# rcelha/rio-rs

Hardware: NVIDIA H100
Metric: placements/sec (higher is better)
Workload: dtype u32

## Files before the change

rio_rs_b200/csrc/k_trie.cu:

```cuda
#include "kernels.cuh"
#include "spec.cuh"
#include "bounded_tail.cuh"

#include <cstdlib>

namespace rio {

namespace {

#define RIO_COUNT_LAUNCH(L) do { if ((L).launch_counter) ++*(L).launch_counter; } while (0)

constexpr int kTrieThreads = 256;
constexpr uint32_t kMaxLevels = 16;

__constant__ uint32_t c_lvl_s0[kMaxLevels];
__constant__ uint32_t c_lvl_m2[kMaxLevels];
__constant__ uint32_t c_lvl_h2[kMaxLevels];

__device__ __forceinline__ uint32_t smem_u32(const void *p) { return (uint32_t)__cvta_generic_to_shared(p); }

__device__ __forceinline__ void stage_blob_tma(void *smem_dst, const void *gsrc, uint32_t bytes, unsigned long long *bar) {
    if (threadIdx.x == 0) {
        asm volatile("mbarrier.init.shared::cta.b64 [%0], 1;" ::"r"(smem_u32(bar)) : "memory");
        asm volatile("fence.mbarrier_init.release.cluster;" ::: "memory");
    }
    __syncthreads();
    if (threadIdx.x == 0) {
        asm volatile("mbarrier.arrive.expect_tx.shared::cta.b64 _, [%0], %1;" ::"r"(smem_u32(bar)), "r"(bytes) : "memory");
        for (uint32_t off = 0; off < bytes; off += 32768u) {
            const uint32_t len = min(32768u, bytes - off);
            asm volatile("cp.async.bulk.shared::cluster.global.mbarrier::complete_tx::bytes [%0], [%1], %2, [%3];"
                         ::"r"(smem_u32(reinterpret_cast<unsigned char *>(smem_dst) + off)),
                           "l"(reinterpret_cast<const unsigned char *>(gsrc) + off), "r"(len), "r"(smem_u32(bar))
                         : "memory");
        }
    }
    uint32_t done = 0;
    while (!done) {
        asm volatile("{\n\t.reg .pred p;\n\tmbarrier.try_wait.parity.shared::cta.b64 p, [%1], %2;\n\tselp.u32 %0, 1, 0, p;\n\t}"
                     : "=r"(done) : "r"(smem_u32(bar)), "r"(0u) : "memory");
    }
}

__device__ __forceinline__ uint32_t walk_step(uint32_t off, uint32_t sel) {
    uint32_t r;
    asm("mad.lo.u32 %0, %1, 2, %2;" : "=r"(r) : "r"(off), "r"(sel));
    return r;
}

template <int BITS>
__device__ __forceinline__ uint32_t trie_leaf_index(ObjHash o, const uint32_t *__restrict__ tab32, uint32_t bits_rt) {
    uint32_t i = 1;
    if (BITS > 0) {
#pragma unroll
        for (int l = 0; l < BITS; l++) {
            const uint32_t u = contest_u(o, c_lvl_s0[l], c_lvl_m2[l], c_lvl_h2[l]);
            i = 2 * i + (u > tab32[i] ? 1u : 0u);
        }
    } else {
        for (uint32_t l = 0; l < bits_rt; l++) {
            const uint32_t u = contest_u(o, c_lvl_s0[l], c_lvl_m2[l], c_lvl_h2[l]);
            i = 2 * i + (u > tab32[i] ? 1u : 0u);
        }
    }
    return i;
}

__device__ __forceinline__ uint32_t trie_resolve_leaf(ObjHash o, uint32_t leaf, const unsigned char *__restrict__ blob) {
    if ((int32_t)leaf > -2) return leaf;
    uint32_t w = leaf;
    for (;;) {
        const unsigned char *p = blob + (w & 0x7FFFFFFFu);
        const uint4 r = *reinterpret_cast<const uint4 *>(p);
        const uint2 nn = *reinterpret_cast<const uint2 *>(p + 16);
        if (contest_u(o, r.x, r.y, r.z) <= r.w) return nn.x;
        if ((int32_t)nn.y >= 0) return nn.y;
        w = nn.y;
    }
}

struct TrieSmem {
    const uint32_t *tab32;
    const unsigned char *blob;
    uint32_t *hist;
};

template <bool SMEM>
__device__ __forceinline__ TrieSmem trie_stage(const TrieDev &t, uint32_t hist_bins) {
    extern __shared__ __align__(128) unsigned char smem_trie[];
    constexpr bool in_smem = SMEM;
    TrieSmem s;
    uint32_t off = 0;
    if (in_smem) {
        s.tab32 = reinterpret_cast<const uint32_t *>(smem_trie);
        s.blob = smem_trie;
        off = t.blob_bytes;
    } else {
        const unsigned char *g = reinterpret_cast<const unsigned char *>(t.blob);
        s.tab32 = reinterpret_cast<const uint32_t *>(g);
        s.blob = g;
    }
    s.hist = reinterpret_cast<uint32_t *>(smem_trie + off);
    for (uint32_t j = threadIdx.x; j < hist_bins; j += blockDim.x) s.hist[j] = 0;
    unsigned long long *bar = reinterpret_cast<unsigned long long *>(smem_trie + off + ((hist_bins * 4u + 15u) & ~15u));
    if (in_smem) stage_blob_tma(smem_trie, t.blob, t.blob_bytes, bar);
    else __syncthreads();
    return s;
}

template <int BITS, int OPT, int MODE, bool SMEM, int MINB = (SMEM ? 5 : 3)>
__global__ void __launch_bounds__(kTrieThreads, MINB)
k_assign_trie(const uint64_t *__restrict__ keys, uint64_t n, TrieDev t, uint32_t *__restrict__ out_idx, uint32_t *__restrict__ counters,
              uint32_t hist_bins, unsigned long long *__restrict__ moved, const __grid_constant__ BoundedTail tail) {
    static_assert(OPT % 2 == 0, "two objects per 128-bit load");
    constexpr bool in_smem = SMEM;
    constexpr int SEG = OPT / 2;
    const uint64_t tile_objs = (uint64_t)kTrieThreads * OPT;
    const uint64_t n_tiles = (n + tile_objs - 1) / tile_objs;
    unsigned long long n_moved = 0;
    ulonglong2 kk[SEG];
    auto load_tile = [&](uint64_t tile) {
        const uint64_t f0 = tile * tile_objs + 2 * threadIdx.x;
        if ((tile + 1) * tile_objs <= n) {
            const ulonglong2 *src = reinterpret_cast<const ulonglong2 *>(keys + f0);
#pragma unroll
            for (int g = 0; g < SEG; g++) kk[g] = __ldg(src + g * kTrieThreads);
            return;
        }
#pragma unroll
        for (int g = 0; g < SEG; g++) {
            const uint64_t f = f0 + (uint64_t)g * (2 * kTrieThreads);
            kk[g] = make_ulonglong2(0, 0);
            if (f + 1 < n) kk[g] = __ldg(reinterpret_cast<const ulonglong2 *>(keys + f));
            else if (f < n) kk[g].x = __ldg(keys + f);
        }
    };
    const TrieSmem s = trie_stage<SMEM>(t, hist_bins);
    asm volatile("griddepcontrol.launch_dependents;" ::: "memory");
    asm volatile("griddepcontrol.wait;" ::: "memory");
    if (blockIdx.x < n_tiles) load_tile(blockIdx.x);
    for (uint64_t tile = blockIdx.x; tile < n_tiles; tile += gridDim.x) {
        const uint64_t base = tile * tile_objs;
        const bool full_tile = base + tile_objs <= n;
        ObjHash o[OPT];
#pragma unroll
        for (int g = 0; g < SEG; g++) {
            o[2 * g] = obj_hash(kk[g].x);
            o[2 * g + 1] = obj_hash(kk[g].y);
        }
        if (tile + gridDim.x < n_tiles) load_tile(tile + gridDim.x);
        uint32_t leaf[OPT];
        if (in_smem) {
            const unsigned char *tb = reinterpret_cast<const unsigned char *>(s.tab32);
            uint32_t off[OPT];
#pragma unroll
            for (int k = 0; k < OPT; k++) off[k] = 4;
            if (BITS > 0) {
                constexpr int TOP = BITS >= 3 ? 3 : 0;
                if (TOP) {
#pragma unroll
                    for (int k = 0; k < OPT; k++) {
                        const bool c0 = contest_u(o[k], c_lvl_s0[0], c_lvl_m2[0], c_lvl_h2[0]) > t.top[1];
                        const bool c1 = contest_u(o[k], c_lvl_s0[1], c_lvl_m2[1], c_lvl_h2[1]) > (c0 ? t.top[3] : t.top[2]);
                        const uint32_t t2 = c0 ? (c1 ? t.top[7] : t.top[6]) : (c1 ? t.top[5] : t.top[4]);
                        const bool c2 = contest_u(o[k], c_lvl_s0[2], c_lvl_m2[2], c_lvl_h2[2]) > t2;
                        off[k] = 32u + (c0 ? 16u : 0u) + (c1 ? 8u : 0u) + (c2 ? 4u : 0u);
                    }
                }
#pragma unroll
                for (int l = TOP; l < BITS; l++) {
#pragma unroll
                    for (int k = 0; k < OPT; k++) {
                        const uint32_t u = contest_u(o[k], c_lvl_s0[l], c_lvl_m2[l], c_lvl_h2[l]);
                        const uint32_t thr = *reinterpret_cast<const uint32_t *>(tb + off[k]);
                        off[k] = walk_step(off[k], u > thr ? 4u : 0u);
                    }
                }
            } else {
                for (uint32_t l = 0; l < t.bits; l++) {
#pragma unroll
                    for (int k = 0; k < OPT; k++) {
                        const uint32_t u = contest_u(o[k], c_lvl_s0[l], c_lvl_m2[l], c_lvl_h2[l]);
                        const uint32_t thr = *reinterpret_cast<const uint32_t *>(tb + off[k]);
                        off[k] = walk_step(off[k], u > thr ? 4u : 0u);
                    }
                }
            }
#pragma unroll
            for (int k = 0; k < OPT; k++) leaf[k] = *reinterpret_cast<const uint32_t *>(tb + off[k]);
        } else {
#pragma unroll
            for (int k = 0; k < OPT; k++) leaf[k] = __ldg(s.tab32 + trie_leaf_index<0>(o[k], s.tab32, t.bits));
        }
        uint32_t nid[OPT];
#pragma unroll
        for (int k = 0; k < OPT; k++) nid[k] = trie_resolve_leaf(o[k], leaf[k], s.blob);
        if (MODE == 0 && full_tile) {
            uint2 *dst = reinterpret_cast<uint2 *>(out_idx + base + 2 * threadIdx.x);
#pragma unroll
            for (int g = 0; g < SEG; g++) dst[g * kTrieThreads] = make_uint2(nid[2 * g], nid[2 * g + 1]);
            if (counters && nid[0] != kNone) {
                if (hist_bins) {
#pragma unroll
                    for (int k = 0; k < OPT; k++) atomicAdd(&s.hist[nid[k]], 1u);
                } else {
#pragma unroll
                    for (int k = 0; k < OPT; k++) atomicAdd(&counters[nid[k]], 1u);
                }
            }
            continue;
        }
#pragma unroll
        for (int g = 0; g < SEG; g++) {
            const uint64_t first = base + (uint64_t)g * (2 * kTrieThreads) + 2 * threadIdx.x;
            if (first >= n) continue;
            const bool two = first + 1 < n;
            if (MODE == 1) {
                uint2 old = make_uint2(kNone, kNone);
                if (two) old = *reinterpret_cast<const uint2 *>(out_idx + first);
                else old.x = out_idx[first];
                const bool c0 = old.x != nid[2 * g], c1 = two && old.y != nid[2 * g + 1];
                if (c0 | c1) {
                    if (two) *reinterpret_cast<uint2 *>(out_idx + first) = make_uint2(nid[2 * g], nid[2 * g + 1]);
                    else out_idx[first] = nid[2 * g];
                }
                n_moved += (unsigned)c0 + (unsigned)c1;
            } else {
                if (two) *reinterpret_cast<uint2 *>(out_idx + first) = make_uint2(nid[2 * g], nid[2 * g + 1]);
                else out_idx[first] = nid[2 * g];
            }
            if (counters) {
                if (hist_bins) {
                    if (nid[2 * g] != kNone) atomicAdd(&s.hist[nid[2 * g]], 1u);
                    if (two && nid[2 * g + 1] != kNone) atomicAdd(&s.hist[nid[2 * g + 1]], 1u);
                } else {
                    if (nid[2 * g] != kNone) atomicAdd(&counters[nid[2 * g]], 1u);
                    if (two && nid[2 * g + 1] != kNone) atomicAdd(&counters[nid[2 * g + 1]], 1u);
                }
            }
        }
    }
    if (MODE == 1) {
#pragma unroll
        for (int sh = 16; sh > 0; sh >>= 1) n_moved += __shfl_xor_sync(0xFFFFFFFFu, n_moved, sh);
        if ((threadIdx.x & 31) == 0 && n_moved) atomicAdd(moved, n_moved);
    }
    if (hist_bins && counters) {
        __syncthreads();
        for (uint32_t j = threadIdx.x; j < hist_bins; j += blockDim.x) { const uint32_t v = s.hist[j]; if (v) atomicAdd(&counters[j], v); }
    }
    if (MODE == 0 && tail.enabled) {
        __shared__ uint32_t s_last;
        __threadfence();
        __syncthreads();
        if (threadIdx.x == 0) s_last = atomicAdd(tail.ticket, 1u) == gridDim.x - 1;
        __syncthreads();
        if (s_last) {
            if (threadIdx.x == 0) *tail.ticket = 0;
            __threadfence();
            exchange_and_check_block(tail, counters);
        }
    }
}

template <bool SMEM>
__global__ void __launch_bounds__(kTrieThreads, 4)
k_assign_trie_sel(const uint64_t *__restrict__ keys, const uint32_t *__restrict__ sel, uint64_t n_sel, TrieDev t, uint32_t *__restrict__ out_idx,
                  uint32_t *__restrict__ counters, uint32_t hist_bins) {
    const TrieSmem s = trie_stage<SMEM>(t, hist_bins);
    for (uint64_t q = (uint64_t)blockIdx.x * blockDim.x + threadIdx.x; q < n_sel; q += (uint64_t)gridDim.x * blockDim.x) {
        const uint32_t oi = __ldg(sel + q);
        const ObjHash o = obj_hash(__ldg(keys + oi));
        const uint32_t i = trie_leaf_index<0>(o, s.tab32, t.bits);
        const uint32_t nid = trie_resolve_leaf(o, s.tab32[i], s.blob);
        out_idx[oi] = nid;
        if (counters && nid != kNone) { if (hist_bins) atomicAdd(&s.hist[nid], 1u); else atomicAdd(&counters[nid], 1u); }
    }
    if (hist_bins && counters) {
        __syncthreads();
        for (uint32_t j = threadIdx.x; j < hist_bins; j += blockDim.x) { const uint32_t v = s.hist[j]; if (v) atomicAdd(&counters[j], v); }
    }
}

template <bool SMEM>
__global__ void __launch_bounds__(kTrieThreads, 4)
k_dir_reassign_trie(DirDev dir, TrieDev t, unsigned long long *__restrict__ moved) {
    const TrieSmem s = trie_stage<SMEM>(t, 0);
    const uint4 *slots = reinterpret_cast<const uint4 *>(dir.slots);
    const uint64_t cap = dir.mask + 1;
    unsigned long long n_moved = 0;
    for (uint64_t i = (uint64_t)blockIdx.x * blockDim.x + threadIdx.x; i < cap; i += (uint64_t)gridDim.x * blockDim.x) {
        const uint4 v = slots[i];
        const unsigned long long key = ((unsigned long long)v.y << 32) | v.x;
        if (key == kEmptyKey || v.z == kNone) continue;
        const ObjHash o = obj_hash(key);
        const uint32_t li = trie_leaf_index<0>(o, s.tab32, t.bits);
        const uint32_t nid = trie_resolve_leaf(o, s.tab32[li], s.blob);
        if (nid != v.z) { reinterpret_cast<uint32_t *>(&dir.slots[i].val)[0] = nid; n_moved++; }
    }
#pragma unroll
    for (int sh = 16; sh > 0; sh >>= 1) n_moved += __shfl_xor_sync(0xFFFFFFFFu, n_moved, sh);
    if ((threadIdx.x & 31) == 0 && n_moved) atomicAdd(moved, n_moved);
}

constexpr uint32_t kTrieSmemBudget = 200u * 1024u;

struct TrieLaunchShape { uint32_t hist_bins; uint32_t in_smem; size_t smem; int ctas_per_sm; };
TrieLaunchShape trie_shape(const TrieDev &t, bool want_hist, uint32_t n_total, int want_ctas) {
    TrieLaunchShape sh{};
    sh.hist_bins = (want_hist && n_total <= 8192) ? n_total : 0;
    const size_t tail = ((size_t)sh.hist_bins * 4 + 15) / 16 * 16 + 16;
    sh.in_smem = (t.blob_bytes + tail <= kTrieSmemBudget) ? 1u : 0u;
    sh.smem = (sh.in_smem ? t.blob_bytes : 0) + tail;
    int c = want_ctas;
    while (c > 1 && (size_t)c * (sh.smem + 1024) > 227u * 1024u) c--;
    sh.ctas_per_sm = c;
    return sh;
}

bool g_lvl_uploaded[64] = {};

}

void trie_upload_level_constants(int device) {
    if (device >= 0 && device < 64 && g_lvl_uploaded[device]) return;
    uint32_t s0[kMaxLevels], m2[kMaxLevels], h2[kMaxLevels];
    for (uint32_t l = 0; l < kMaxLevels; l++) {
        const ContestRec r = contest_rec(level_seed(l));
        s0[l] = r.s0; m2[l] = r.m2; h2[l] = r.h2;
    }
    cudaMemcpyToSymbol(c_lvl_s0, s0, sizeof s0);
    cudaMemcpyToSymbol(c_lvl_m2, m2, sizeof m2);
    cudaMemcpyToSymbol(c_lvl_h2, h2, sizeof h2);
    if (device >= 0 && device < 64) g_lvl_uploaded[device] = true;
}

uint64_t trie_wave_objects(int sm_count) { return (uint64_t)sm_count * 5 * kTrieThreads * 4; }

#define RIO_TRIE_LAUNCH(KERNEL, GRID, SMEM, ...)                                                                       \
    do {                                                                                                               \
        static bool attr_set[64] = {};    \
        int dev__ = 0;                                                                                                 \
        cudaGetDevice(&dev__);                                                                                         \
        if (dev__ < 0 || dev__ >= 64 || !attr_set[dev__]) {                                                            \
            cudaFuncSetAttribute(KERNEL, cudaFuncAttributeMaxDynamicSharedMemorySize, (int)kTrieSmemBudget + 1024);    \
            if (dev__ >= 0 && dev__ < 64) attr_set[dev__] = true;                                                      \
        }                                                                                                              \
        KERNEL<<<(GRID), kTrieThreads, (SMEM), L.stream>>>(__VA_ARGS__);                                               \
    } while (0)

#define RIO_TRIE_LAUNCH_PDL(KERNEL, GRID, SMEM, ...)                                                                   \
    do {                                                                                                               \
        static bool attr_set[64] = {};                                                                                 \
        static const bool pdl = [] { const char *e = getenv("RIO_TRIE_PDL"); return !(e && e[0] == '0'); }();          \
        int dev__ = 0;                                                                                                 \
        cudaGetDevice(&dev__);                                                                                         \
        if (dev__ < 0 || dev__ >= 64 || !attr_set[dev__]) {                                                            \
            cudaFuncSetAttribute(KERNEL, cudaFuncAttributeMaxDynamicSharedMemorySize, (int)kTrieSmemBudget + 1024);    \
            if (dev__ >= 0 && dev__ < 64) attr_set[dev__] = true;                                                      \
        }                                                                                                              \
        cudaLaunchConfig_t cfg__ = {};                                                                                 \
        cfg__.gridDim = dim3((unsigned)(GRID)); cfg__.blockDim = dim3(kTrieThreads);                                   \
        cfg__.dynamicSmemBytes = (SMEM); cfg__.stream = L.stream;                                                      \
        cudaLaunchAttribute at__[1];                                                                                   \
        at__[0].id = cudaLaunchAttributeProgrammaticStreamSerialization;                                               \
        at__[0].val.programmaticStreamSerializationAllowed = 1;                                                        \
        cfg__.attrs = at__; cfg__.numAttrs = pdl ? 1 : 0;                                                              \
        cudaLaunchKernelEx(&cfg__, KERNEL, __VA_ARGS__);                                                               \
    } while (0)

void launch_assign_trie(const Launch &L, const uint64_t *d_keys, uint64_t n, const TrieDev &t, uint32_t *d_out_idx, uint32_t *d_counters,
                        const uint32_t *d_sel, uint64_t n_sel, uint32_t n_total, const BoundedTail *tail) {
    BoundedTail no_tail{};
    const BoundedTail &tl = tail ? *tail : no_tail;
    const uint64_t n_work = d_sel ? n_sel : n;
    if (!n_work) return;
    if (d_sel) {
        const TrieLaunchShape sh = trie_shape(t, d_counters != nullptr, n_total, 4);
        const uint64_t blocks = (n_work + kTrieThreads - 1) / kTrieThreads, cap = (uint64_t)L.sm_count * sh.ctas_per_sm;
        const int grid = (int)(blocks < cap ? blocks : cap);
        if (sh.in_smem) RIO_TRIE_LAUNCH(k_assign_trie_sel<true>, grid, sh.smem, d_keys, d_sel, n_work, t, d_out_idx, d_counters, sh.hist_bins);
        else RIO_TRIE_LAUNCH(k_assign_trie_sel<false>, grid, sh.smem, d_keys, d_sel, n_work, t, d_out_idx, d_counters, sh.hist_bins);
    } else {
        constexpr int OPT = 4;
#ifdef RIO_ASSIGN_TUNING
        if (const char *tn = getenv("RIO_TRIE_TUNE")) {
            const int code = atoi(tn);
            auto go = [&](auto kern, int opt, int minb) {
                const TrieLaunchShape sh2 = trie_shape(t, d_counters != nullptr, n_total, minb);
                const uint64_t tiles2 = (n_work + (uint64_t)kTrieThreads * opt - 1) / ((uint64_t)kTrieThreads * opt), cap2 = (uint64_t)L.sm_count * sh2.ctas_per_sm;
                cudaFuncSetAttribute(kern, cudaFuncAttributeMaxDynamicSharedMemorySize, (int)kTrieSmemBudget + 1024);
                kern<<<(int)(tiles2 < cap2 ? tiles2 : cap2), kTrieThreads, sh2.smem, L.stream>>>(d_keys, n_work, t, d_out_idx, d_counters, sh2.hist_bins, nullptr, tl);
            };
            bool done = true;
            switch (code) {
                case 25: go(k_assign_trie<12, 2, 0, true, 5>, 2, 5); break;
                case 28: go(k_assign_trie<12, 2, 0, true, 8>, 2, 8); break;
                case 44: go(k_assign_trie<12, 4, 0, true, 4>, 4, 4); break;
                case 45: go(k_assign_trie<12, 4, 0, true, 5>, 4, 5); break;
                case 63: go(k_assign_trie<12, 6, 0, true, 3>, 6, 3); break;
                case 64: go(k_assign_trie<12, 6, 0, true, 4>, 6, 4); break;
                case 83: go(k_assign_trie<12, 8, 0, true, 3>, 8, 3); break;
                default: done = false;
            }
            if (done && t.bits == 12) { RIO_COUNT_LAUNCH(L); return; }
        }
#endif
        const TrieLaunchShape sh = trie_shape(t, d_counters != nullptr, n_total, 5);
        uint64_t cap = (uint64_t)L.sm_count * sh.ctas_per_sm;
        if (L.spare_ctas > 0 && cap > (uint64_t)L.spare_ctas + 1) cap -= (uint64_t)L.spare_ctas;
        const uint64_t tiles = (n_work + (uint64_t)kTrieThreads * OPT - 1) / ((uint64_t)kTrieThreads * OPT);
        const int grid = (int)(tiles < cap ? tiles : cap);
        unsigned long long *no_moved = nullptr;
        if (!sh.in_smem) RIO_TRIE_LAUNCH_PDL((k_assign_trie<0, OPT, 0, false>), grid, sh.smem, d_keys, n_work, t, d_out_idx, d_counters, sh.hist_bins, no_moved, tl);
        else if (t.bits == 12) RIO_TRIE_LAUNCH_PDL((k_assign_trie<12, OPT, 0, true>), grid, sh.smem, d_keys, n_work, t, d_out_idx, d_counters, sh.hist_bins, no_moved, tl);
        else RIO_TRIE_LAUNCH_PDL((k_assign_trie<0, OPT, 0, true>), grid, sh.smem, d_keys, n_work, t, d_out_idx, d_counters, sh.hist_bins, no_moved, tl);
    }
    RIO_COUNT_LAUNCH(L);
}

void launch_reassign_trie(const Launch &L, const uint64_t *d_keys, uint64_t n, const TrieDev &t, uint32_t *d_idx, uint32_t *d_counters,
                          uint32_t n_total, unsigned long long *d_moved) {
    if (!n) return;
    constexpr int OPT = 4;
 const TrieLaunchShape sh = trie_shape(t, d_counters != nullptr, n_total, 5);
    const uint64_t tiles = (n + (uint64_t)kTrieThreads * OPT - 1) / ((uint64_t)kTrieThreads * OPT), cap = (uint64_t)L.sm_count * sh.ctas_per_sm;
    const int grid = (int)(tiles < cap ? tiles : cap);
    if (!sh.in_smem) RIO_TRIE_LAUNCH((k_assign_trie<0, OPT, 1, false>), grid, sh.smem, d_keys, n, t, d_idx, d_counters, sh.hist_bins, d_moved, BoundedTail{});
    else if (t.bits == 12) RIO_TRIE_LAUNCH((k_assign_trie<12, OPT, 1, true>), grid, sh.smem, d_keys, n, t, d_idx, d_counters, sh.hist_bins, d_moved, BoundedTail{});
    else RIO_TRIE_LAUNCH((k_assign_trie<0, OPT, 1, true>), grid, sh.smem, d_keys, n, t, d_idx, d_counters, sh.hist_bins, d_moved, BoundedTail{});
    RIO_COUNT_LAUNCH(L);
}

void launch_dir_reassign_trie(const Launch &L, const DirDev &dir, const TrieDev &t, unsigned long long *d_moved) {
    const TrieLaunchShape sh = trie_shape(t, false, 0, 4);
    const uint64_t blocks = (dir.mask + 1 + kTrieThreads - 1) / kTrieThreads, cap = (uint64_t)L.sm_count * sh.ctas_per_sm;
    const int grid = (int)(blocks < cap ? blocks : cap);
    if (sh.in_smem) RIO_TRIE_LAUNCH(k_dir_reassign_trie<true>, grid, sh.smem, dir, t, d_moved);
    else RIO_TRIE_LAUNCH(k_dir_reassign_trie<false>, grid, sh.smem, dir, t, d_moved);
    RIO_COUNT_LAUNCH(L);
}

}
```

Measured before the change: 148.3 billion.

## Replicate mid trie levels per lane in smem to kill bank conflicts; use 1024-thread CTAs

Trie levels 6-9 are copied into shared memory replicated 32-wide, one copy per lane. Lookups at those levels then hit each lane's own bank instead of colliding on a few hot nodes. The kernel now runs 1024-thread CTAs at one CTA per SM. The compare switches to >= with h2-1 so a carry-based descend instruction can be used, and the chain resolve becomes a batched loop across objects. The costs are extra smem for the replicas, a copy step at kernel start, and lower CTA-level occupancy; the launch API also gains a rep argument.

```diff
diff --git a/rio_rs_b200/csrc/k_trie.cu b/rio_rs_b200/csrc/k_trie.cu
--- a/rio_rs_b200/csrc/k_trie.cu
+++ b/rio_rs_b200/csrc/k_trie.cu
@@ -2,6 +2,7 @@
 #include "spec.cuh"
 #include "bounded_tail.cuh"
 
+#include <algorithm>
 #include <cstdlib>
 
 namespace rio {
@@ -11,7 +12,13 @@
 #define RIO_COUNT_LAUNCH(L) do { if ((L).launch_counter) ++*(L).launch_counter; } while (0)
 
 constexpr int kTrieThreads = 256;
+constexpr int kWalkThreads = 1024;
+constexpr int kWalkCtas = 1;
 constexpr uint32_t kMaxLevels = 16;
+constexpr uint32_t kRepFirst = 6;
+constexpr uint32_t kRepMax = 4;
+__host__ __device__ constexpr uint32_t rep_bytes(uint32_t levels) { return ((1u << (kRepFirst + levels)) - (1u << kRepFirst)) * 128u; }
+constexpr int default_rep(int bits) { return bits <= (int)kRepFirst ? 0 : bits - (int)kRepFirst < (int)kRepMax ? bits - (int)kRepFirst : (int)kRepMax; }
 
 __constant__ uint32_t c_lvl_s0[kMaxLevels];
 __constant__ uint32_t c_lvl_m2[kMaxLevels];
@@ -42,9 +49,9 @@
     }
 }
 
-__device__ __forceinline__ uint32_t walk_step(uint32_t off, uint32_t sel) {
+__device__ __forceinline__ uint32_t descend(uint32_t i, uint32_t u1, uint32_t t3) {
     uint32_t r;
-    asm("mad.lo.u32 %0, %1, 2, %2;" : "=r"(r) : "r"(off), "r"(sel));
+    asm("{\n\t.reg .u32 d;\n\tsub.cc.u32 d, %1, %2;\n\taddc.u32 %0, %3, %3;\n\t}" : "=r"(r) : "r"(u1), "r"(t3), "r"(i));
     return r;
 }
 
@@ -54,13 +61,13 @@
     if (BITS > 0) {
 #pragma unroll
         for (int l = 0; l < BITS; l++) {
-            const uint32_t u = contest_u(o, c_lvl_s0[l], c_lvl_m2[l], c_lvl_h2[l]);
-            i = 2 * i + (u > tab32[i] ? 1u : 0u);
+            const uint32_t u1 = contest_u(o, c_lvl_s0[l], c_lvl_m2[l], c_lvl_h2[l]);
+            i = 2 * i + (u1 >= tab32[i] ? 1u : 0u);
         }
     } else {
         for (uint32_t l = 0; l < bits_rt; l++) {
-            const uint32_t u = contest_u(o, c_lvl_s0[l], c_lvl_m2[l], c_lvl_h2[l]);
-            i = 2 * i + (u > tab32[i] ? 1u : 0u);
+            const uint32_t u1 = contest_u(o, c_lvl_s0[l], c_lvl_m2[l], c_lvl_h2[l]);
+            i = 2 * i + (u1 >= tab32[i] ? 1u : 0u);
         }
     }
     return i;
@@ -79,43 +86,58 @@
     }
 }
 
+extern __shared__ __align__(128) unsigned char smem_trie[];
+
+__device__ __forceinline__ uint32_t lds_u32(uint32_t byte_off) { return *reinterpret_cast<const uint32_t *>(smem_trie + byte_off); }
+
 struct TrieSmem {
     const uint32_t *tab32;
     const unsigned char *blob;
     uint32_t *hist;
+    uint32_t rep_lane;
 };
 
 template <bool SMEM>
-__device__ __forceinline__ TrieSmem trie_stage(const TrieDev &t, uint32_t hist_bins) {
-    extern __shared__ __align__(128) unsigned char smem_trie[];
+__device__ __forceinline__ TrieSmem trie_stage(const TrieDev &t, uint32_t hist_bins, uint32_t rep = 0) {
     constexpr bool in_smem = SMEM;
     TrieSmem s;
     uint32_t off = 0;
     if (in_smem) {
         s.tab32 = reinterpret_cast<const uint32_t *>(smem_trie);
         s.blob = smem_trie;
-        off = t.blob_bytes;
+        off = t.blob_bytes + rep_bytes(rep);
     } else {
         const unsigned char *g = reinterpret_cast<const unsigned char *>(t.blob);
         s.tab32 = reinterpret_cast<const uint32_t *>(g);
         s.blob = g;
     }
+    s.rep_lane = t.blob_bytes + (threadIdx.x & 31u) * 4u - (1u << kRepFirst) * 128u;
     s.hist = reinterpret_cast<uint32_t *>(smem_trie + off);
     for (uint32_t j = threadIdx.x; j < hist_bins; j += blockDim.x) s.hist[j] = 0;
     unsigned long long *bar = reinterpret_cast<unsigned long long *>(smem_trie + off + ((hist_bins * 4u + 15u) & ~15u));
     if (in_smem) stage_blob_tma(smem_trie, t.blob, t.blob_bytes, bar);
     else __syncthreads();
+    if (in_smem && rep) {
+        uint4 *dst = reinterpret_cast<uint4 *>(smem_trie + t.blob_bytes);
+        const uint32_t *src = s.tab32 + (1u << kRepFirst);
+        for (uint32_t q = threadIdx.x; q < rep_bytes(rep) / 16u; q += blockDim.x) {
+            const uint32_t v = src[q >> 3];
+            dst[q] = make_uint4(v, v, v, v);
+        }
+        __syncthreads();
+    }
     return s;
 }
 
-template <int BITS, int OPT, int MODE, bool SMEM, int MINB = (SMEM ? 5 : 3)>
-__global__ void __launch_bounds__(kTrieThreads, MINB)
+template <int BITS, int OPT, int MODE, bool SMEM, int NT = kWalkThreads, int MINB = kWalkCtas, int REP = default_rep(BITS)>
+__global__ void __launch_bounds__(NT, MINB)
 k_assign_trie(const uint64_t *__restrict__ keys, uint64_t n, TrieDev t, uint32_t *__restrict__ out_idx, uint32_t *__restrict__ counters,
-              uint32_t hist_bins, unsigned long long *__restrict__ moved, const __grid_constant__ BoundedTail tail) {
+              uint32_t hist_bins, uint32_t rep, unsigned long long *__restrict__ moved, const __grid_constant__ BoundedTail tail) {
     static_assert(OPT % 2 == 0, "two objects per 128-bit load");
+    static_assert(BITS == 0 || BITS >= 3 + REP, "the unrolled walk takes levels 0-2 from the parameter bank");
     constexpr bool in_smem = SMEM;
     constexpr int SEG = OPT / 2;
-    const uint64_t tile_objs = (uint64_t)kTrieThreads * OPT;
+    const uint64_t tile_objs = (uint64_t)NT * OPT;
     const uint64_t n_tiles = (n + tile_objs - 1) / tile_objs;
     unsigned long long n_moved = 0;
     ulonglong2 kk[SEG];
@@ -124,18 +146,18 @@
         if ((tile + 1) * tile_objs <= n) {
             const ulonglong2 *src = reinterpret_cast<const ulonglong2 *>(keys + f0);
 #pragma unroll
-            for (int g = 0; g < SEG; g++) kk[g] = __ldg(src + g * kTrieThreads);
+            for (int g = 0; g < SEG; g++) kk[g] = __ldg(src + g * NT);
             return;
         }
 #pragma unroll
         for (int g = 0; g < SEG; g++) {
-            const uint64_t f = f0 + (uint64_t)g * (2 * kTrieThreads);
+            const uint64_t f = f0 + (uint64_t)g * (2 * NT);
             kk[g] = make_ulonglong2(0, 0);
             if (f + 1 < n) kk[g] = __ldg(reinterpret_cast<const ulonglong2 *>(keys + f));
             else if (f < n) kk[g].x = __ldg(keys + f);
         }
     };
-    const TrieSmem s = trie_stage<SMEM>(t, hist_bins);
+    const TrieSmem s = trie_stage<SMEM>(t, hist_bins, BITS > 0 ? (uint32_t)REP : rep);
     asm volatile("griddepcontrol.launch_dependents;" ::: "memory");
     asm volatile("griddepcontrol.wait;" ::: "memory");
     if (blockIdx.x < n_tiles) load_tile(blockIdx.x);
@@ -149,56 +171,63 @@
             o[2 * g + 1] = obj_hash(kk[g].y);
         }
         if (tile + gridDim.x < n_tiles) load_tile(tile + gridDim.x);
-        uint32_t leaf[OPT];
+        uint32_t nid[OPT];
         if (in_smem) {
-            const unsigned char *tb = reinterpret_cast<const unsigned char *>(s.tab32);
-            uint32_t off[OPT];
-#pragma unroll
-            for (int k = 0; k < OPT; k++) off[k] = 4;
+            uint32_t i[OPT];
+#pragma unroll
+            for (int k = 0; k < OPT; k++) i[k] = 1;
             if (BITS > 0) {
-                constexpr int TOP = BITS >= 3 ? 3 : 0;
-                if (TOP) {
+#pragma unroll
+                for (int k = 0; k < OPT; k++) {
+                    const bool c0 = contest_u(o[k], c_lvl_s0[0], c_lvl_m2[0], c_lvl_h2[0]) >= t.top[1];
+                    const bool c1 = contest_u(o[k], c_lvl_s0[1], c_lvl_m2[1], c_lvl_h2[1]) >= (c0 ? t.top[3] : t.top[2]);
+                    const uint32_t t2 = c0 ? (c1 ? t.top[7] : t.top[6]) : (c1 ? t.top[5] : t.top[4]);
+                    i[k] = descend(4u + (c0 ? 2u : 0u) + (c1 ? 1u : 0u), contest_u(o[k], c_lvl_s0[2], c_lvl_m2[2], c_lvl_h2[2]), t2);
+                }
+#pragma unroll
+                for (int l = 3; l < BITS; l++) {
+                    const bool copied = l >= (int)kRepFirst && l < (int)kRepFirst + REP;
 #pragma unroll
                     for (int k = 0; k < OPT; k++) {
-                        const bool c0 = contest_u(o[k], c_lvl_s0[0], c_lvl_m2[0], c_lvl_h2[0]) > t.top[1];
-                        const bool c1 = contest_u(o[k], c_lvl_s0[1], c_lvl_m2[1], c_lvl_h2[1]) > (c0 ? t.top[3] : t.top[2]);
-                        const uint32_t t2 = c0 ? (c1 ? t.top[7] : t.top[6]) : (c1 ? t.top[5] : t.top[4]);
-                        const bool c2 = contest_u(o[k], c_lvl_s0[2], c_lvl_m2[2], c_lvl_h2[2]) > t2;
-                        off[k] = 32u + (c0 ? 16u : 0u) + (c1 ? 8u : 0u) + (c2 ? 4u : 0u);
-                    }
-                }
-#pragma unroll
-                for (int l = TOP; l < BITS; l++) {
-#pragma unroll
-                    for (int k = 0; k < OPT; k++) {
-                        const uint32_t u = contest_u(o[k], c_lvl_s0[l], c_lvl_m2[l], c_lvl_h2[l]);
-                        const uint32_t thr = *reinterpret_cast<const uint32_t *>(tb + off[k]);
-                        off[k] = walk_step(off[k], u > thr ? 4u : 0u);
+                        const uint32_t u1 = contest_u(o[k], c_lvl_s0[l], c_lvl_m2[l], c_lvl_h2[l]);
+                        i[k] = descend(i[k], u1, lds_u32(copied ? s.rep_lane + (i[k] << 7) : i[k] << 2));
                     }
                 }
             } else {
                 for (uint32_t l = 0; l < t.bits; l++) {
+                    const bool copied = l - kRepFirst < rep;
 #pragma unroll
                     for (int k = 0; k < OPT; k++) {
-                        const uint32_t u = contest_u(o[k], c_lvl_s0[l], c_lvl_m2[l], c_lvl_h2[l]);
-                        const uint32_t thr = *reinterpret_cast<const uint32_t *>(tb + off[k]);
-                        off[k] = walk_step(off[k], u > thr ? 4u : 0u);
+                        const uint32_t u1 = contest_u(o[k], c_lvl_s0[l], c_lvl_m2[l], c_lvl_h2[l]);
+                        i[k] = descend(i[k], u1, lds_u32(copied ? s.rep_lane + (i[k] << 7) : i[k] << 2));
                     }
                 }
             }
 #pragma unroll
-            for (int k = 0; k < OPT; k++) leaf[k] = *reinterpret_cast<const uint32_t *>(tb + off[k]);
+            for (int k = 0; k < OPT; k++) nid[k] = lds_u32(i[k] << 2);
         } else {
 #pragma unroll
-            for (int k = 0; k < OPT; k++) leaf[k] = __ldg(s.tab32 + trie_leaf_index<0>(o[k], s.tab32, t.bits));
-        }
-        uint32_t nid[OPT];
-#pragma unroll
-        for (int k = 0; k < OPT; k++) nid[k] = trie_resolve_leaf(o[k], leaf[k], s.blob);
+            for (int k = 0; k < OPT; k++) nid[k] = __ldg(s.tab32 + trie_leaf_index<0>(o[k], s.tab32, t.bits));
+        }
+        for (;;) {
+            bool chained = false;
+#pragma unroll
+            for (int k = 0; k < OPT; k++) chained |= (int32_t)nid[k] < -1;
+            if (!chained) break;
+#pragma unroll
+            for (int k = 0; k < OPT; k++) {
+                if ((int32_t)nid[k] < -1) {
+                    const unsigned char *p = s.blob + (nid[k] & 0x7FFFFFFFu);
+                    const uint4 r = *reinterpret_cast<const uint4 *>(p);
+                    const uint2 nn = *reinterpret_cast<const uint2 *>(p + 16);
+                    nid[k] = contest_u(o[k], r.x, r.y, r.z) <= r.w ? nn.x : nn.y;
+                }
+            }
+        }
         if (MODE == 0 && full_tile) {
             uint2 *dst = reinterpret_cast<uint2 *>(out_idx + base + 2 * threadIdx.x);
 #pragma unroll
-            for (int g = 0; g < SEG; g++) dst[g * kTrieThreads] = make_uint2(nid[2 * g], nid[2 * g + 1]);
+            for (int g = 0; g < SEG; g++) dst[g * NT] = make_uint2(nid[2 * g], nid[2 * g + 1]);
             if (counters && nid[0] != kNone) {
                 if (hist_bins) {
 #pragma unroll
@@ -212,7 +241,7 @@
         }
 #pragma unroll
         for (int g = 0; g < SEG; g++) {
-            const uint64_t first = base + (uint64_t)g * (2 * kTrieThreads) + 2 * threadIdx.x;
+            const uint64_t first = base + (uint64_t)g * (2 * NT) + 2 * threadIdx.x;
             if (first >= n) continue;
             const bool two = first + 1 < n;
             if (MODE == 1) {
@@ -305,15 +334,19 @@
 
 constexpr uint32_t kTrieSmemBudget = 200u * 1024u;
 
-struct TrieLaunchShape { uint32_t hist_bins; uint32_t in_smem; size_t smem; int ctas_per_sm; };
-TrieLaunchShape trie_shape(const TrieDev &t, bool want_hist, uint32_t n_total, int want_ctas) {
+struct TrieLaunchShape { uint32_t hist_bins; uint32_t in_smem; uint32_t rep; size_t smem; int ctas_per_sm; };
+TrieLaunchShape trie_shape(const TrieDev &t, bool want_hist, uint32_t n_total, int want_ctas, uint32_t max_rep = 0) {
     TrieLaunchShape sh{};
     sh.hist_bins = (want_hist && n_total <= 8192) ? n_total : 0;
     const size_t tail = ((size_t)sh.hist_bins * 4 + 15) / 16 * 16 + 16;
     sh.in_smem = (t.blob_bytes + tail <= kTrieSmemBudget) ? 1u : 0u;
-    sh.smem = (sh.in_smem ? t.blob_bytes : 0) + tail;
+    const size_t staged = (sh.in_smem ? t.blob_bytes : 0) + tail;
     int c = want_ctas;
-    while (c > 1 && (size_t)c * (sh.smem + 1024) > 227u * 1024u) c--;
+    while (c > 1 && (size_t)c * (staged + 1024) > 227u * 1024u) c--;
+    uint32_t r = (sh.in_smem && t.bits > kRepFirst) ? std::min(t.bits - kRepFirst, max_rep) : 0u;
+    while (r && (staged + rep_bytes(r) > kTrieSmemBudget || (size_t)c * (staged + rep_bytes(r) + 1024) > 227u * 1024u)) r--;
+    sh.rep = r;
+    sh.smem = staged + rep_bytes(r);
     sh.ctas_per_sm = c;
     return sh;
 }
@@ -327,7 +360,7 @@
     uint32_t s0[kMaxLevels], m2[kMaxLevels], h2[kMaxLevels];
     for (uint32_t l = 0; l < kMaxLevels; l++) {
         const ContestRec r = contest_rec(level_seed(l));
-        s0[l] = r.s0; m2[l] = r.m2; h2[l] = r.h2;
+        s0[l] = r.s0; m2[l] = r.m2; h2[l] = r.h2 - 1u;
     }
     cudaMemcpyToSymbol(c_lvl_s0, s0, sizeof s0);
     cudaMemcpyToSymbol(c_lvl_m2, m2, sizeof m2);
@@ -335,9 +368,9 @@
     if (device >= 0 && device < 64) g_lvl_uploaded[device] = true;
 }
 
-uint64_t trie_wave_objects(int sm_count) { return (uint64_t)sm_count * 5 * kTrieThreads * 4; }
-
-#define RIO_TRIE_LAUNCH(KERNEL, GRID, SMEM, ...)                                                                       \
+uint64_t trie_wave_objects(int sm_count) { return (uint64_t)sm_count * kWalkCtas * kWalkThreads * 4; }
+
+#define RIO_TRIE_LAUNCH(KERNEL, GRID, NT, SMEM, ...)                                                                   \
     do {                                                                                                               \
         static bool attr_set[64] = {};    \
         int dev__ = 0;                                                                                                 \
@@ -346,10 +379,10 @@
             cudaFuncSetAttribute(KERNEL, cudaFuncAttributeMaxDynamicSharedMemorySize, (int)kTrieSmemBudget + 1024);    \
             if (dev__ >= 0 && dev__ < 64) attr_set[dev__] = true;                                                      \
         }                                                                                                              \
-        KERNEL<<<(GRID), kTrieThreads, (SMEM), L.stream>>>(__VA_ARGS__);                                               \
+        KERNEL<<<(GRID), (NT), (SMEM), L.stream>>>(__VA_ARGS__);                                                       \
     } while (0)
 
-#define RIO_TRIE_LAUNCH_PDL(KERNEL, GRID, SMEM, ...)                                                                   \
+#define RIO_TRIE_LAUNCH_PDL(KERNEL, GRID, NT, SMEM, ...)                                                               \
     do {                                                                                                               \
         static bool attr_set[64] = {};                                                                                 \
         static const bool pdl = [] { const char *e = getenv("RIO_TRIE_PDL"); return !(e && e[0] == '0'); }();          \
@@ -360,7 +393,7 @@
             if (dev__ >= 0 && dev__ < 64) attr_set[dev__] = true;                                                      \
         }                                                                                                              \
         cudaLaunchConfig_t cfg__ = {};                                                                                 \
-        cfg__.gridDim = dim3((unsigned)(GRID)); cfg__.blockDim = dim3(kTrieThreads);                                   \
+        cfg__.gridDim = dim3((unsigned)(GRID)); cfg__.blockDim = dim3(NT);                                             \
         cfg__.dynamicSmemBytes = (SMEM); cfg__.stream = L.stream;                                                      \
         cudaLaunchAttribute at__[1];                                                                                   \
         at__[0].id = cudaLaunchAttributeProgrammaticStreamSerialization;                                               \
@@ -379,42 +412,41 @@
         const TrieLaunchShape sh = trie_shape(t, d_counters != nullptr, n_total, 4);
         const uint64_t blocks = (n_work + kTrieThreads - 1) / kTrieThreads, cap = (uint64_t)L.sm_count * sh.ctas_per_sm;
         const int grid = (int)(blocks < cap ? blocks : cap);
-        if (sh.in_smem) RIO_TRIE_LAUNCH(k_assign_trie_sel<true>, grid, sh.smem, d_keys, d_sel, n_work, t, d_out_idx, d_counters, sh.hist_bins);
-        else RIO_TRIE_LAUNCH(k_assign_trie_sel<false>, grid, sh.smem, d_keys, d_sel, n_work, t, d_out_idx, d_counters, sh.hist_bins);
+        if (sh.in_smem) RIO_TRIE_LAUNCH(k_assign_trie_sel<true>, grid, kTrieThreads, sh.smem, d_keys, d_sel, n_work, t, d_out_idx, d_counters, sh.hist_bins);
+        else RIO_TRIE_LAUNCH(k_assign_trie_sel<false>, grid, kTrieThreads, sh.smem, d_keys, d_sel, n_work, t, d_out_idx, d_counters, sh.hist_bins);
     } else {
         constexpr int OPT = 4;
+        unsigned long long *no_moved = nullptr;
 #ifdef RIO_ASSIGN_TUNING
         if (const char *tn = getenv("RIO_TRIE_TUNE")) {
             const int code = atoi(tn);
-            auto go = [&](auto kern, int opt, int minb) {
-                const TrieLaunchShape sh2 = trie_shape(t, d_counters != nullptr, n_total, minb);
-                const uint64_t tiles2 = (n_work + (uint64_t)kTrieThreads * opt - 1) / ((uint64_t)kTrieThreads * opt), cap2 = (uint64_t)L.sm_count * sh2.ctas_per_sm;
+            auto go = [&](auto kern, int opt, int nt, int minb, uint32_t rep) {
+                const TrieLaunchShape sh2 = trie_shape(t, d_counters != nullptr, n_total, minb, rep);
+                if (sh2.rep != rep) return false;
+                const uint64_t tiles2 = (n_work + (uint64_t)nt * opt - 1) / ((uint64_t)nt * opt), cap2 = (uint64_t)L.sm_count * sh2.ctas_per_sm;
                 cudaFuncSetAttribute(kern, cudaFuncAttributeMaxDynamicSharedMemorySize, (int)kTrieSmemBudget + 1024);
-                kern<<<(int)(tiles2 < cap2 ? tiles2 : cap2), kTrieThreads, sh2.smem, L.stream>>>(d_keys, n_work, t, d_out_idx, d_counters, sh2.hist_bins, nullptr, tl);
+                kern<<<(int)(tiles2 < cap2 ? tiles2 : cap2), nt, sh2.smem, L.stream>>>(d_keys, n_work, t, d_out_idx, d_counters, sh2.hist_bins, rep, no_moved, tl);
+                return true;
             };
-            bool done = true;
-            switch (code) {
-                case 25: go(k_assign_trie<12, 2, 0, true, 5>, 2, 5); break;
-                case 28: go(k_assign_trie<12, 2, 0, true, 8>, 2, 8); break;
-                case 44: go(k_assign_trie<12, 4, 0, true, 4>, 4, 4); break;
-                case 45: go(k_assign_trie<12, 4, 0, true, 5>, 4, 5); break;
-                case 63: go(k_assign_trie<12, 6, 0, true, 3>, 6, 3); break;
-                case 64: go(k_assign_trie<12, 6, 0, true, 4>, 6, 4); break;
-                case 83: go(k_assign_trie<12, 8, 0, true, 3>, 8, 3); break;
-                default: done = false;
-            }
-            if (done && t.bits == 12) { RIO_COUNT_LAUNCH(L); return; }
+            bool done = false;
+            if (t.bits == 12) switch (code) {
+                case 41: done = go(k_assign_trie<12, 4, 0, true, 1024, 1, 4>, 4, 1024, 1, 4); break;
+                case 42: done = go(k_assign_trie<12, 4, 0, true, 640, 2, 3>, 4, 640, 2, 3); break;
+                case 61: done = go(k_assign_trie<12, 6, 0, true, 1024, 1, 4>, 6, 1024, 1, 4); break;
+                case 81: done = go(k_assign_trie<12, 8, 0, true, 1024, 1, 4>, 8, 1024, 1, 4); break;
+                default: break;
+            }
+            if (done) { RIO_COUNT_LAUNCH(L); return; }
         }
 #endif
-        const TrieLaunchShape sh = trie_shape(t, d_counters != nullptr, n_total, 5);
+        const TrieLaunchShape sh = trie_shape(t, d_counters != nullptr, n_total, kWalkCtas, kRepMax);
         uint64_t cap = (uint64_t)L.sm_count * sh.ctas_per_sm;
         if (L.spare_ctas > 0 && cap > (uint64_t)L.spare_ctas + 1) cap -= (uint64_t)L.spare_ctas;
-        const uint64_t tiles = (n_work + (uint64_t)kTrieThreads * OPT - 1) / ((uint64_t)kTrieThreads * OPT);
+        const uint64_t tiles = (n_work + (uint64_t)kWalkThreads * OPT - 1) / ((uint64_t)kWalkThreads * OPT);
         const int grid = (int)(tiles < cap ? tiles : cap);
-        unsigned long long *no_moved = nullptr;
-        if (!sh.in_smem) RIO_TRIE_LAUNCH_PDL((k_assign_trie<0, OPT, 0, false>), grid, sh.smem, d_keys, n_work, t, d_out_idx, d_counters, sh.hist_bins, no_moved, tl);
-        else if (t.bits == 12) RIO_TRIE_LAUNCH_PDL((k_assign_trie<12, OPT, 0, true>), grid, sh.smem, d_keys, n_work, t, d_out_idx, d_counters, sh.hist_bins, no_moved, tl);
-        else RIO_TRIE_LAUNCH_PDL((k_assign_trie<0, OPT, 0, true>), grid, sh.smem, d_keys, n_work, t, d_out_idx, d_counters, sh.hist_bins, no_moved, tl);
+        if (!sh.in_smem) RIO_TRIE_LAUNCH_PDL((k_assign_trie<0, OPT, 0, false>), grid, kWalkThreads, sh.smem, d_keys, n_work, t, d_out_idx, d_counters, sh.hist_bins, 0u, no_moved, tl);
+        else if (t.bits == 12 && sh.rep == kRepMax) RIO_TRIE_LAUNCH_PDL((k_assign_trie<12, OPT, 0, true>), grid, kWalkThreads, sh.smem, d_keys, n_work, t, d_out_idx, d_counters, sh.hist_bins, sh.rep, no_moved, tl);
+        else RIO_TRIE_LAUNCH_PDL((k_assign_trie<0, OPT, 0, true>), grid, kWalkThreads, sh.smem, d_keys, n_work, t, d_out_idx, d_counters, sh.hist_bins, sh.rep, no_moved, tl);
     }
     RIO_COUNT_LAUNCH(L);
 }
@@ -423,12 +455,12 @@
                           uint32_t n_total, unsigned long long *d_moved) {
     if (!n) return;
     constexpr int OPT = 4;
- const TrieLaunchShape sh = trie_shape(t, d_counters != nullptr, n_total, 5);
-    const uint64_t tiles = (n + (uint64_t)kTrieThreads * OPT - 1) / ((uint64_t)kTrieThreads * OPT), cap = (uint64_t)L.sm_count * sh.ctas_per_sm;
+    const TrieLaunchShape sh = trie_shape(t, d_counters != nullptr, n_total, kWalkCtas, kRepMax);
+    const uint64_t tiles = (n + (uint64_t)kWalkThreads * OPT - 1) / ((uint64_t)kWalkThreads * OPT), cap = (uint64_t)L.sm_count * sh.ctas_per_sm;
     const int grid = (int)(tiles < cap ? tiles : cap);
-    if (!sh.in_smem) RIO_TRIE_LAUNCH((k_assign_trie<0, OPT, 1, false>), grid, sh.smem, d_keys, n, t, d_idx, d_counters, sh.hist_bins, d_moved, BoundedTail{});
-    else if (t.bits == 12) RIO_TRIE_LAUNCH((k_assign_trie<12, OPT, 1, true>), grid, sh.smem, d_keys, n, t, d_idx, d_counters, sh.hist_bins, d_moved, BoundedTail{});
-    else RIO_TRIE_LAUNCH((k_assign_trie<0, OPT, 1, true>), grid, sh.smem, d_keys, n, t, d_idx, d_counters, sh.hist_bins, d_moved, BoundedTail{});
+    if (!sh.in_smem) RIO_TRIE_LAUNCH((k_assign_trie<0, OPT, 1, false>), grid, kWalkThreads, sh.smem, d_keys, n, t, d_idx, d_counters, sh.hist_bins, 0u, d_moved, BoundedTail{});
+    else if (t.bits == 12 && sh.rep == kRepMax) RIO_TRIE_LAUNCH((k_assign_trie<12, OPT, 1, true>), grid, kWalkThreads, sh.smem, d_keys, n, t, d_idx, d_counters, sh.hist_bins, sh.rep, d_moved, BoundedTail{});
+    else RIO_TRIE_LAUNCH((k_assign_trie<0, OPT, 1, true>), grid, kWalkThreads, sh.smem, d_keys, n, t, d_idx, d_counters, sh.hist_bins, sh.rep, d_moved, BoundedTail{});
     RIO_COUNT_LAUNCH(L);
 }
 
@@ -436,8 +468,8 @@
     const TrieLaunchShape sh = trie_shape(t, false, 0, 4);
     const uint64_t blocks = (dir.mask + 1 + kTrieThreads - 1) / kTrieThreads, cap = (uint64_t)L.sm_count * sh.ctas_per_sm;
     const int grid = (int)(blocks < cap ? blocks : cap);
-    if (sh.in_smem) RIO_TRIE_LAUNCH(k_dir_reassign_trie<true>, grid, sh.smem, dir, t, d_moved);
-    else RIO_TRIE_LAUNCH(k_dir_reassign_trie<false>, grid, sh.smem, dir, t, d_moved);
+    if (sh.in_smem) RIO_TRIE_LAUNCH(k_dir_reassign_trie<true>, grid, kTrieThreads, sh.smem, dir, t, d_moved);
+    else RIO_TRIE_LAUNCH(k_dir_reassign_trie<false>, grid, kTrieThreads, sh.smem, dir, t, d_moved);
     RIO_COUNT_LAUNCH(L);
 }
 
```

Result: faster. 159.8 billion, median of 6 (+7.8%).
